# broadinstitute/gatk-bwamem-jni

Hardware: AMD Instinct MI355X
Metric: 150bp reads aligned/sec vs GRCh38-scale reference (1/2/4/8 MI355X) (higher is better)
Workload: dtype u8/int32/int64; 1 GPU; 10000000 x 150bp single-end synthetic reads per GPU vs synthetic GRCh38-scale genome (3100000000 bp, 24 contigs, 5% diverged repeats), full index in HBM; reads_per_gpu=10000000, read_len=150, genome_bp=3100000000, genome=iid, response_bytes=542940344, parallelism=read-sharded x1, no collectives, hip_hw_queues=4, paired_end=False

## Files before the change

gatk-bwamem-jni_amd/csrc/k_seed.hip:

```cpp
#include "dev_common.h"
#include "wave_ops.h"
#include "kernels.h"

DEV uint32_t mask16(int n)
{
    n = n < 0 ? 0 : n > 16 ? 16 : n;
    return (uint32_t)(0x5555555500000000ull >> (n << 1));
}
DEV void cnt_word_m(uint32_t x, uint32_t m, uint32_t& c1, uint32_t& c2, uint32_t& c3)
{
    const uint32_t lo = x & m, hi = (x >> 1) & m;
    c3 += __popc(hi & lo);
    c2 += __popc(hi & ~lo);
    c1 += __popc(~hi & lo);
}
DEV void extend_sm(const DevIndex& ix, uint64_t x0, uint64_t x1, uint64_t size, int c, bool is_back, uint64_t& o0, uint64_t& o1, uint64_t& osz)
{
    const uint64_t xa = is_back ? x0 : x1, xb = is_back ? x1 : x0;
    const uint64_t k = xa - 1, l = xa - 1 + size;
    const uint64_t kk = k - (k >= ix.primary), ll = l - (l >= ix.primary);
    const uint64_t bk = kk >> 6, bl = ll >> 6;
    const uint4* pk = ix.occ + 2 * bk;
    const uint4* pl = ix.occ + 2 * bl;
    const uint4 ck = pk[0], sk = pk[1], cl = pl[0], sl = pl[1];
// ... 291 lines not shown
            i = sx - 1; c = c0;
            if (!walk && (cmask & ~gone & short_mask)) st = S_PRB0;
            else if (lo >= nf) END_SEARCH();
            else { rd = wr = nf - 1; st = S_BWD; }
        }
        if (emit) MEM_PUSH(em0, ems, emi);
        if (ovf) FINISH();
        if (fin) {
            tv.n_intv[r] = ovf ? 0 : mem_n;
            if (ovf) atomicOr(tv.err, ERR_INTV_CAP);
        }
    }
#undef QAT
#undef FINISH
#undef MEM_PUSH
#undef PUSH_IK
#undef END_SEARCH
#undef BEGIN_BWD
    unsigned long long tot = n_ext;
    for (int o = 32; o > 0; o >>= 1) tot += __shfl_down(tot, o);
    if (lane == 0) { count_add(&tv.cnt->n_ext, tot); }
}

__global__ void k_seed_fin(MemOpt opt, TileView tv)
{
    const int r = blockIdx.x * blockDim.x + threadIdx.x;
    if (r >= tv.n_reads) return;
    Intv* a = tv.intv + (size_t)r * tv.intv_cap;
    const int n = tv.n_intv[r];
    for (int i = 1; i < n; ++i) {
        Intv t = a[i];
        int j = i;
        while (j > 0 && a[j - 1].info > t.info) { a[j] = a[j - 1]; --j; }
        a[j] = t;
    }
    int n_seeds = 0, l_rep = 0, b = 0, e = 0;
    int32_t* iso = tv.intv_seed_off + (size_t)r * tv.intv_cap;
    for (int i = 0; i < n; ++i) {
        const Intv p = a[i];
        const int sb = (int)(p.info >> 32), se = (int)(uint32_t)p.info;
        iso[i] = n_seeds;
        {
            int64_t step = p.size > (uint64_t)(int64_t)opt.max_occ ? (int64_t)(p.size / (uint64_t)opt.max_occ) : 1;
            int64_t c = ((int64_t)p.size + step - 1) / step;
            n_seeds += (int)(c < opt.max_occ ? c : opt.max_occ);
        }
        if (p.size <= (uint64_t)(int64_t)opt.max_occ) continue;
        if (sb > e) { l_rep += e - b; b = sb; e = se; }
        else e = e > se ? e : se;
    }
    l_rep += e - b;
    tv.n_seeds[r] = n_seeds;
    tv.l_rep[r] = l_rep;
}

__global__ void __launch_bounds__(1024) k_scan(const int32_t* in, int64_t* out, int n)
{
    __shared__ int64_t wtot[2][16];
    const int t = threadIdx.x, lane = t & 63, wv = t >> 6;
    int64_t carry = 0;
    int ph = 0;
    for (int base = 0; base < n; base += 4096, ph ^= 1) {
        const int i0 = base + t * 4;
        int v0 = 0, v1 = 0, v2 = 0, v3 = 0;
        if (i0 + 3 < n) { const int4 q = *(const int4*)(in + i0); v0 = q.x; v1 = q.y; v2 = q.z; v3 = q.w; }
        else { if (i0 < n) v0 = in[i0]; if (i0 + 1 < n) v1 = in[i0 + 1]; if (i0 + 2 < n) v2 = in[i0 + 2]; }
        const int64_t sum = (int64_t)v0 + v1 + v2 + v3;
        int64_t incl = sum;
        for (int o = 1; o < 64; o <<= 1) { int64_t u = __shfl_up(incl, o); if (lane >= o) incl += u; }
        if (lane == 63) wtot[ph][wv] = incl;
        __syncthreads();
        int64_t pre = carry, tot = 0;
        for (int w = 0; w < 16; ++w) { const int64_t x = wtot[ph][w]; if (w < wv) pre += x; tot += x; }
        int64_t run = pre + incl - sum;
        if (i0 < n) out[i0] = run;
        run += v0; if (i0 + 1 < n) out[i0 + 1] = run;
        run += v1; if (i0 + 2 < n) out[i0 + 2] = run;
        run += v2; if (i0 + 3 < n) out[i0 + 3] = run;
        carry += tot;
    }
    if (t == 0) out[n] = carry;
}

DEV int64_t block_excl_scan_256(int64_t v, int64_t* lds4, int64_t& total)
{
    const int lane = threadIdx.x & 63, wv = threadIdx.x >> 6;
    int64_t incl = v;
    for (int o = 1; o < 64; o <<= 1) { int64_t u = __shfl_up(incl, o); if (lane >= o) incl += u; }
    if (lane == 63) lds4[wv] = incl;
    __syncthreads();
    int64_t pre = 0; total = 0;
    for (int w = 0; w < 4; ++w) { const int64_t x = lds4[w]; if (w < wv) pre += x; total += x; }
    __syncthreads();
    return pre + incl - v;
}
__global__ void __launch_bounds__(256) k_scan_part(const int32_t* in, int n, int64_t* part)
{
    __shared__ int64_t w4[4];
    const int i0 = blockIdx.x * 4096 + threadIdx.x * 16;
    int64_t sum = 0;
    for (int k = 0; k < 16; k += 4) {
        const int i = i0 + k;
        if (i + 3 < n) { const int4 q = *(const int4*)(in + i); sum += (int64_t)q.x + q.y + q.z + q.w; }
        else for (int j = i; j < n && j < i + 4; ++j) sum += in[j];
    }
    int64_t tot;
    (void)block_excl_scan_256(sum, w4, tot);
    if (threadIdx.x == 0) part[blockIdx.x] = tot;
}
__global__ void __launch_bounds__(64) k_scan_top(int64_t* part, int nb, int64_t* total_out)
{
    const int lane = threadIdx.x;
    int64_t carry = 0;
    for (int base = 0; base < nb; base += 64) {
        const int i = base + lane;
        const int64_t v = i < nb ? part[i] : 0;
        int64_t incl = v;
        for (int o = 1; o < 64; o <<= 1) { int64_t u = __shfl_up(incl, o); if (lane >= o) incl += u; }
        if (i < nb) part[i] = carry + incl - v;
        carry += __shfl(incl, 63);
    }
    if (lane == 0) *total_out = carry;
}
template <bool FUSED>
__global__ void __launch_bounds__(256) k_scan_apply(const int32_t* in, int n, const int64_t* part, int64_t* out)
{
    __shared__ int64_t w4[4];
    const int i0 = blockIdx.x * 4096 + threadIdx.x * 16;
    int v[16];
    int64_t sum = 0;
    for (int k = 0; k < 16; ++k) { v[k] = i0 + k < n ? in[i0 + k] : 0; sum += v[k]; }
    int64_t tot, base;
    if (FUSED) {
        int64_t mine = 0, before;
        for (int b = threadIdx.x; b < (int)blockIdx.x; b += 256) mine += part[b];
        (void)block_excl_scan_256(mine, w4, before);
        base = before;
    } else base = part[blockIdx.x];
    int64_t run = base + block_excl_scan_256(sum, w4, tot);
    for (int k = 0; k < 16; ++k) { if (i0 + k < n) out[i0 + k] = run; run += v[k]; }
    if (FUSED && blockIdx.x == gridDim.x - 1 && threadIdx.x == 0) out[n] = base + tot;
}

DEV int order_bin(int n_seeds) { return n_seeds <= 0 ? 31 : __clz(n_seeds); }
__global__ void __launch_bounds__(256) k_order_count(const int32_t* n_seeds, int n, int32_t* bins)
{
    __shared__ int32_t h[32];
    if (threadIdx.x < 32) h[threadIdx.x] = 0;
    __syncthreads();
    const int r = blockIdx.x * blockDim.x + threadIdx.x;
    if (r < n) atomicAdd(&h[order_bin(n_seeds[r])], 1);
    __syncthreads();
    if (threadIdx.x < 32 && h[threadIdx.x]) atomicAdd(&bins[threadIdx.x], h[threadIdx.x]);
}
__global__ void k_order_offsets(int32_t* bins)
{
    if (threadIdx.x == 0 && blockIdx.x == 0) { int acc = 0; for (int b = 0; b < 32; ++b) { bins[32 + b] = acc; acc += bins[b]; } }
}
__global__ void __launch_bounds__(256) k_order_scatter(const int32_t* n_seeds, int n, int32_t* bins, int32_t* order)
{
    __shared__ int32_t h[32], base[32];
    if (threadIdx.x < 32) h[threadIdx.x] = 0;
    __syncthreads();
    const int r = blockIdx.x * blockDim.x + threadIdx.x;
    int b = 0, rank = 0;
    if (r < n) { b = order_bin(n_seeds[r]); rank = atomicAdd(&h[b], 1); }
    __syncthreads();
    if (threadIdx.x < 32) base[threadIdx.x] = h[threadIdx.x] ? atomicAdd(&bins[32 + threadIdx.x], h[threadIdx.x]) : 0;
    __syncthreads();
    if (r < n) order[base[b] + rank] = r;
}
void launch_order(hipStream_t st, const int32_t* n_seeds, int n, int32_t* bins64, int32_t* order)
{
    if (n <= 0) return;
    (void)hipMemsetAsync(bins64, 0, 64 * sizeof(int32_t), st);
    hipLaunchKernelGGL(k_order_count, dim3((n + 255) / 256), dim3(256), 0, st, n_seeds, n, bins64);
    hipLaunchKernelGGL(k_order_offsets, dim3(1), dim3(64), 0, st, bins64);
    hipLaunchKernelGGL(k_order_scatter, dim3((n + 255) / 256), dim3(256), 0, st, n_seeds, n, bins64, order);
}

DEV uint32_t zero_byte_mask(uint32_t w) { return ~(((w & 0x7f7f7f7fu) + 0x7f7f7f7fu) | w | 0x7f7f7f7fu); }
DEV void nul_words(const uint8_t* seq, int64_t n_bytes, int64_t b0, uint32_t m[4])
{
    const uint4 q = *(const uint4*)(seq + b0);
    const uint32_t w[4] = { q.x, q.y, q.z, q.w };
    for (int k = 0; k < 4; ++k) {
        const int64_t left = n_bytes - (b0 + 4 * k);
        uint32_t z = zero_byte_mask(w[k]);
        if (left < 4) z = left <= 0 ? 0u : z & (0xffffffffu >> (8 * (4 - (int)left)));
        m[k] = z;
    }
}
__global__ void __launch_bounds__(256) k_nul_count(const uint8_t* seq, int64_t n_bytes, int32_t* cnt)
{
    __shared__ int64_t w4[4];
    const int64_t b0 = (int64_t)blockIdx.x * 4096 + threadIdx.x * 16;
    uint32_t m[4] = { 0, 0, 0, 0 };
    if (b0 < n_bytes) nul_words(seq, n_bytes, b0, m);
    int64_t tot;
    (void)block_excl_scan_256((int64_t)(__popc(m[0]) + __popc(m[1]) + __popc(m[2]) + __popc(m[3])), w4, tot);
    if (threadIdx.x == 0) cnt[blockIdx.x] = (int32_t)tot;
}
__global__ void __launch_bounds__(256) k_nul_write(const uint8_t* seq, int64_t n_bytes, const int64_t* blk_off, int nb, int64_t* off, int64_t n_reads_max, int64_t* n_found)
{
    __shared__ int64_t w4[4];
    const int64_t b0 = (int64_t)blockIdx.x * 4096 + threadIdx.x * 16;
    uint32_t m[4] = { 0, 0, 0, 0 };
    if (b0 < n_bytes) nul_words(seq, n_bytes, b0, m);
    int64_t tot;
    int64_t k = blk_off[blockIdx.x] + block_excl_scan_256((int64_t)(__popc(m[0]) + __popc(m[1]) + __popc(m[2]) + __popc(m[3])), w4, tot);
    for (int w = 0; w < 4; ++w)
        for (int j = 0; j < 4; ++j)
            if (m[w] >> (8 * j + 7) & 1) { if (k < n_reads_max) off[k + 1] = b0 + 4 * w + j + 1; ++k; }
    if (blockIdx.x == 0 && threadIdx.x == 0) *n_found = blk_off[nb];
}

__global__ void k_sa(DevIndex ix, MemOpt opt, TileView tv, int64_t n_occ)
{
    int64_t g = (int64_t)blockIdx.x * blockDim.x + threadIdx.x;
    uint32_t n_lf = 0, n_sa = 0;
    if (g < n_occ) {
        int lo = 0, hi = tv.n_reads;
        while (hi - lo > 1) { int mid = (lo + hi) >> 1; if (tv.seed_off[mid] <= g) lo = mid; else hi = mid; }
        int r = lo;
        int local = (int)(g - tv.seed_off[r]);
        const int32_t* iso = tv.intv_seed_off + (size_t)r * tv.intv_cap;
        int n = tv.n_intv[r];
        lo = 0; hi = n;
        while (hi - lo > 1) { int mid = (lo + hi) >> 1; if (iso[mid] <= local) lo = mid; else hi = mid; }
        Intv p = tv.intv[(size_t)r * tv.intv_cap + lo];
        int64_t step = p.size > (uint64_t)(int64_t)opt.max_occ ? (int64_t)(p.size / (uint64_t)opt.max_occ) : 1;
        int64_t k = (int64_t)(local - iso[lo]) * step;
        Seed s;
        s.rbeg = (int64_t)sa_lookup(ix, p.x0 + (uint64_t)k, n_lf); ++n_sa;
        s.qbeg = (int32_t)(p.info >> 32);
        s.len = s.score = (int32_t)((uint32_t)p.info - (uint32_t)(p.info >> 32));
        s.next = -1;
        tv.seeds[g] = s;
        tv.seed_rid[g] = bns_intv2rid(ix, s.rbeg, s.rbeg + s.len);
    }
    unsigned long long a = n_lf, b = n_sa;
    for (int o = 32; o > 0; o >>= 1) { a += __shfl_down(a, o); b += __shfl_down(b, o); }
    if ((threadIdx.x & 63) == 0) { count_add(&tv.cnt->n_lf, a); count_add(&tv.cnt->n_sa, b); }
}

__global__ void k_sa_densify(DevIndex ix, const uint64_t* sa_src, uint64_t n_src, int src_intv, uint32_t* lo, uint8_t* hi, int32_t* err)
{
    const uint64_t t = (uint64_t)blockIdx.x * blockDim.x + threadIdx.x;
    if (t >= n_src) return;
    uint64_t k = t * (uint64_t)src_intv, v = sa_src[t];
    lo[k >> ix.sa_shift] = (uint32_t)v; hi[k >> ix.sa_shift] = (uint8_t)(v >> 32);
    if (ix.sa_intv == src_intv) return;
    if (t == 0) v = ix.seq_len;
    const uint64_t smask = (uint64_t)src_intv - 1, dmask = (uint64_t)ix.sa_intv - 1;
    for (uint64_t step = 0; ; ++step) {
        if (step > ix.seq_len) { atomicOr(err, ERR_SCRATCH); return; }
        k = lf_step(ix, k);
        if (!(k & smask)) return;
        --v;
        if (!(k & dmask)) { lo[k >> ix.sa_shift] = (uint32_t)v; hi[k >> ix.sa_shift] = (uint8_t)(v >> 32); }
    }
}

void launch_sa_densify(hipStream_t st, const DevIndex& ix, const uint64_t* sa_src, uint64_t n_src, int src_intv, uint32_t* lo, uint8_t* hi, int32_t* err)
{
    hipLaunchKernelGGL(k_sa_densify, dim3((unsigned)((n_src + 255) / 256)), dim3(256), 0, st, ix, sa_src, n_src, src_intv, lo, hi, err);
}

__global__ void k_build_occ64(const uint32_t* bwt, uint64_t n_blocks, uint4* occ)
{
    uint64_t b = (uint64_t)blockIdx.x * blockDim.x + threadIdx.x;
    if (b >= n_blocks) return;
    const uint32_t* blk = bwt + (b >> 1 << 4);
    const uint64_t* cnt = (const uint64_t*)blk;
    const uint32_t* sym = blk + 8 + ((b & 1) << 2);
    uint32_t c1 = 0, c2 = 0, c3 = 0;
    if (b & 1) for (int i = 0; i < 4; ++i) cnt_word(blk[8 + i], 16, c1, c2, c3);
    const uint64_t C = cnt[1] + c1, G = cnt[2] + c2, T = cnt[3] + c3;
    uint4 c, s;
    c.x = (uint32_t)C; c.y = (uint32_t)G; c.z = (uint32_t)T;
    c.w = (uint32_t)(C >> 32 & 0xff) | (uint32_t)(G >> 32 & 0xff) << 8 | (uint32_t)(T >> 32 & 0xff) << 16;
    s.x = sym[0]; s.y = sym[1]; s.z = sym[2]; s.w = sym[3];
    occ[2 * b] = c; occ[2 * b + 1] = s;
}

void launch_build_occ64(hipStream_t st, const uint32_t* bwt, uint64_t n_blocks, uint4* occ)
{
    hipLaunchKernelGGL(k_build_occ64, dim3((unsigned)((n_blocks + 255) / 256)), dim3(256), 0, st, bwt, n_blocks, occ);
}

__global__ void k_unpack_pac(const uint8_t* pac, int64_t start, int64_t n, uint8_t* dst)
{
    int64_t i = (int64_t)blockIdx.x * blockDim.x + threadIdx.x;
    const int64_t stride = (int64_t)gridDim.x * blockDim.x;
    for (; i < n; i += stride) dst[i] = (uint8_t)pac_base(pac, start + i);
}
void launch_unpack_pac(hipStream_t st, const DevIndex& ix, int64_t start, int64_t n, uint8_t* dst)
{
    if (n <= 0) return;
    int64_t nb = (n + 255) / 256;
    if (nb > 65536) nb = 65536;
    hipLaunchKernelGGL(k_unpack_pac, dim3((unsigned)nb), dim3(256), 0, st, ix.pac, start, n, dst);
}

void launch_encode(hipStream_t st, uint8_t* seq, int64_t n_bytes)
{
    if (n_bytes <= 0) return;
    int64_t nb = (n_bytes + 255) / 256;
    if (nb > 8192) nb = 8192;
    hipLaunchKernelGGL(k_encode, dim3((unsigned)nb), dim3(256), 0, st, seq, n_bytes);
}
void launch_seed(hipStream_t st, const DevIndex& ix, const MemOpt& opt, const TileView& tv)
{
    if (tv.n_reads <= 0) return;
    const int n_cu = ix.n_cu > 0 ? ix.n_cu : 256;
    int K = 16, wpc = 0, refill_min = 4;
    { const char* e = getenv("BWAMEM_HIP_SEED_REFILL"); if (e && atoi(e) > 0) refill_min = atoi(e); }
    { const char* e = getenv("BWAMEM_HIP_SEED_K"); if (e && atoi(e) > 0) K = atoi(e); }
    { const char* e = getenv("BWAMEM_HIP_SEED_WPC"); if (e && atoi(e) > 0) wpc = atoi(e); }
    while (K & (K - 1)) K &= K - 1;
    const size_t qbytes = (size_t)64 * 4 * (((size_t)tv.max_len + 7) / 8);
    const bool ldsq = qbytes <= 24576;
    int narrow = ix.seq_len < (1ull << 35) && tv.max_len < 1023;
    { const char* e = getenv("BWAMEM_HIP_SEED_NARROW"); if (e) narrow = narrow && atoi(e) != 0; }
    const size_t lds = (size_t)(narrow ? 5 * K * 32 : 3 * K * 64) * 4 + (size_t)SEED_EL_CAP * 64 * 4 + (ldsq ? qbytes : 0) + 16;
    if (!wpc) { wpc = (int)((size_t)(160 * 1024) / ((lds + 1023) & ~(size_t)1023)); wpc = wpc < 1 ? 1 : wpc > 16 ? 16 : wpc; }
    const int groups = (tv.n_reads + 63) / 64;
    int grid = groups < n_cu * wpc ? groups : n_cu * wpc;
    if (tv.smem_groups > 0 && grid > tv.smem_groups) grid = tv.smem_groups;
    TileView tvs = tv;
    { const char* e = getenv("BWAMEM_HIP_SEED_PROBE"); if (e && e[0] == '0' && !e[1]) tvs.seed_no_probe = 1; }
    if (ldsq) hipLaunchKernelGGL(k_seed<true>, dim3(grid), dim3(64), lds, st, ix, opt, tvs, K, refill_min, narrow);
    else hipLaunchKernelGGL(k_seed<false>, dim3(grid), dim3(64), lds, st, ix, opt, tvs, K, refill_min, narrow);
    hipLaunchKernelGGL(k_seed_fin, dim3((tv.n_reads + 255) / 256), dim3(256), 0, st, opt, tv);
}
size_t scan_tmp_bytes(int64_t n) { return (size_t)((n + 4095) / 4096 + 2) * 8; }
static int scan_knob(const char* name, int dflt) { const char* e = getenv(name); return e && atoi(e) > 0 ? atoi(e) : dflt; }
void launch_scan(hipStream_t st, const int32_t* in, int64_t* out, int n, int64_t* tmp)
{
    const int single_max = scan_knob("BWAMEM_HIP_SCAN_SINGLE_MAX", 8192), fused_max = scan_knob("BWAMEM_HIP_SCAN_FUSED_MAX", 2048);
    if (n <= single_max || !tmp) { hipLaunchKernelGGL(k_scan, dim3(1), dim3(1024), 0, st, in, out, n); return; }
    const int nb = (n + 4095) / 4096;
    hipLaunchKernelGGL(k_scan_part, dim3(nb), dim3(256), 0, st, in, n, tmp);
    if (nb <= fused_max) { hipLaunchKernelGGL(k_scan_apply<true>, dim3(nb), dim3(256), 0, st, in, n, (const int64_t*)tmp, out); return; }
    hipLaunchKernelGGL(k_scan_top, dim3(1), dim3(64), 0, st, tmp, nb, out + n);
    hipLaunchKernelGGL(k_scan_apply<false>, dim3(nb), dim3(256), 0, st, in, n, (const int64_t*)tmp, out);
}
size_t nul_tmp_bytes(int64_t n_bytes) { const size_t nb = (size_t)((n_bytes + 15) / 4096 + 2); return nb * 4 + 128 + (nb + 1) * 8 + scan_tmp_bytes((int64_t)nb); }
void launch_nul_offsets(hipStream_t st, const uint8_t* seq, int64_t n_bytes, int64_t* off, int64_t n_reads_max, int64_t* n_found, void* tmp)
{
    const int nb = (int)((n_bytes + 4095) / 4096);
    int32_t* cnt = (int32_t*)tmp;
    int64_t* blk_off = (int64_t*)((char*)tmp + (((size_t)(nb + 2) * 4 + 63) & ~(size_t)63));
    int64_t* scan_tmp = blk_off + nb + 1;
    (void)hipMemsetAsync(off, 0, 8, st);
    if (nb <= 0) { (void)hipMemsetAsync(n_found, 0, 8, st); return; }
    hipLaunchKernelGGL(k_nul_count, dim3(nb), dim3(256), 0, st, seq, n_bytes, cnt);
    launch_scan(st, cnt, blk_off, nb, scan_tmp);
    hipLaunchKernelGGL(k_nul_write, dim3(nb), dim3(256), 0, st, seq, n_bytes, (const int64_t*)blk_off, nb, off, n_reads_max, n_found);
}
void launch_sa(hipStream_t st, const DevIndex& ix, const MemOpt& opt, const TileView& tv, int64_t n_occ)
{
    if (n_occ <= 0) return;
    hipLaunchKernelGGL(k_sa, dim3((unsigned)((n_occ + 255) / 256)), dim3(256), 0, st, ix, opt, tv, n_occ);
}
```

gatk-bwamem-jni_amd/csrc/kernels.h:

```cpp
#pragma once
#include <hip/hip_runtime.h>
#include "bwamem_types.h"
#include "bam_encode.h"
#include "bam_sort.h"
#include "bam_dup.h"
#include "fastq_parse.h"

void launch_build_occ64(hipStream_t st, const uint32_t* bwt, uint64_t n_blocks, uint4* occ);
void launch_sa_densify(hipStream_t st, const DevIndex& ix, const uint64_t* sa_src, uint64_t n_src, int src_intv, uint32_t* lo, uint8_t* hi, int32_t* err);
void launch_encode(hipStream_t st, uint8_t* seq, int64_t n_bytes);
void launch_unpack_pac(hipStream_t st, const DevIndex& ix, int64_t start, int64_t n, uint8_t* dst);
void launch_seed(hipStream_t st, const DevIndex& ix, const MemOpt& opt, const TileView& tv);
size_t scan_tmp_bytes(int64_t n);
void launch_scan(hipStream_t st, const int32_t* in, int64_t* out, int n, int64_t* tmp);
void launch_order(hipStream_t st, const int32_t* n_seeds, int n, int32_t* bins64, int32_t* order);
size_t nul_tmp_bytes(int64_t n_bytes);
void launch_nul_offsets(hipStream_t st, const uint8_t* seq, int64_t n_bytes, int64_t* off, int64_t n_reads_max, int64_t* n_found, void* tmp);
void launch_sa(hipStream_t st, const DevIndex& ix, const MemOpt& opt, const TileView& tv, int64_t n_occ);
void launch_chain(hipStream_t st, const DevIndex& ix, const MemOpt& opt, const TileView& tv, Chain* chain_store);
bool rescore_needed(const MemOpt& opt, const TileView& tv);
void launch_rescore(hipStream_t st, const DevIndex& ix, const MemOpt& opt, const TileView& tv, void* jobs, void* results, int32_t* first_num, int32_t* cnt, int cap);
size_t extend_lds_bytes(const MemOpt& opt, int max_len);
void launch_extend(hipStream_t st, const DevIndex& ix, const MemOpt& opt, const TileView& tv);
void launch_post1(hipStream_t st, const DevIndex& ix, const MemOpt& opt, const TileView& tv);
void launch_final_prep(hipStream_t st, const DevIndex& ix, const MemOpt& opt, const TileView& tv);
size_t gcigar_slab_bytes(const MemOpt& opt, int max_len);
int gcigar_slab_grid(const DevIndex& ix, int n_jobs);
void launch_gcigar(hipStream_t st, const DevIndex& ix, const MemOpt& opt, const TileView& tv, int n_jobs, const void* jobs, void* outs, uint32_t* cig_pool, int cig_cap,
                   uint8_t* zpool, unsigned long long zpool_cap, unsigned long long* zpool_cur, uint8_t* slabs, size_t slab_bytes, int* queue);
void launch_final_se(hipStream_t st, const DevIndex& ix, const MemOpt& opt, const TileView& tv, const void* job_out, const uint32_t* job_cig, int cig_cap);
void launch_pack(hipStream_t st, const TileView& tv, uint8_t* dst);
void launch_bam_size(hipStream_t st, const BamTile& t);
void launch_bam_emit(hipStream_t st, const BamTile& t);
void launch_qual_check(hipStream_t st, const uint8_t* raw, const uint8_t* qual, const int64_t* raw_off, int n_reads, int32_t* err);
void launch_mate_names(hipStream_t st, const uint8_t* names, const int64_t* name_off, int n_pairs, int32_t* err);
void launch_fastq_count(hipStream_t st, const uint8_t* text, int64_t n, int32_t* counts);
void launch_fastq_starts(hipStream_t st, const FastqText& t);
void launch_fastq_records(hipStream_t st, const FastqText& t, const FastqOut& o);
void launch_fastq_copy(hipStream_t st, const FastqText& t, const FastqOut& o, int max_len);
int bgzf_grid(int n_cu, int64_t n_blocks);
size_t bgzf_token_bytes(int grid);
void launch_bgzf_deflate(hipStream_t st, const uint8_t* src, int64_t n, int n_blocks, int grid, uint8_t* slots, int32_t* sizes, uint32_t* tokens);
void launch_bgzf_gather(hipStream_t st, const uint8_t* slots, const int32_t* sizes, const int64_t* off, int n_blocks, bool with_eof, uint8_t* out);
void launch_sort_bits(hipStream_t st, const uint64_t* keys, int64_t n, int32_t* bits);
void launch_sort_hist(hipStream_t st, const uint64_t* keys, int64_t n, int byte, int32_t* hist);
void launch_sort_scatter(hipStream_t st, const uint64_t* keys, const uint32_t* idx, int64_t n, int byte, const int64_t* off, uint64_t* keys_out, uint32_t* idx_out);
void launch_bamrec_count(hipStream_t st, const uint8_t* bam, const int64_t* bam_off, int n_reads, int32_t* counts, int32_t* bits, int32_t* err);
void launch_bamrec_keys(hipStream_t st, const uint8_t* bam, const int64_t* bam_off, int n_reads, const int64_t* first, uint64_t* keys, int64_t* src_off, int32_t* sizes);
void launch_bamrec_sizes(hipStream_t st, const uint32_t* idx, const int32_t* sizes, int n, int32_t* out);
void launch_bamrec_gather(hipStream_t st, const uint8_t* src, const int64_t* src_off, const uint32_t* idx, const int64_t* dst_off, int n_rec, int64_t total, uint8_t* dst);
void launch_bai_records(hipStream_t st, const BaiView& v);
void launch_bai_mark(hipStream_t st, const uint64_t* keys, const uint32_t* idx, int n, int32_t* start);
void launch_bai_chunks(hipStream_t st, const uint64_t* keys, const uint32_t* idx, int n, const int32_t* start, const int64_t* cid, const int64_t* rec_off,
                       const int64_t* member_off, int64_t coffset0, BaiChunk* out);
void launch_bai_windows(hipStream_t st, const int32_t* win, int n_win, int n_rec, const int64_t* rec_off, const int64_t* member_off, int64_t coffset0, uint64_t* out);
void launch_dup_entries(hipStream_t st, const DupView& v);
void launch_dup_scores(hipStream_t st, const DupView& v, int max_len);
void launch_dup_score_keys(hipStream_t st, const DupView& v, uint64_t* frag_key, uint64_t* pair_key);
void launch_dup_gather(hipStream_t st, const uint64_t* src, const uint32_t* idx, int n, uint64_t* out);
void launch_dup_decide(hipStream_t st, const uint64_t* keys, const uint32_t* idx, const uint64_t* second, int n, const uint8_t* is_paired, uint8_t* dup);
void launch_dup_flags(hipStream_t st, const DupView& v);

void launch_pestat_cand(hipStream_t st, const DevIndex& ix, const MemOpt& opt, const TileView& tv, int8_t* cand_dir, int64_t* cand_is);
void launch_pe_caps(hipStream_t st, const MemOpt& opt, const TileView& tv, int32_t* caps);
void launch_pe_copy_regs(hipStream_t st, const TileView& tv, const AlnReg* src, const int64_t* src_off, AlnReg* dst, const int64_t* dst_off, const int32_t* n_regs);
void launch_pe_pair(hipStream_t st, const DevIndex& ix, const MemOpt& opt, const TileView& tv, AlnReg* regs, const int64_t* reg_off,
                    int32_t* n_regs, int32_t* ints, void* vpool, void* keys, uint8_t* scratch, int64_t scratch_per_pair, int cap_h, int cap_b, int cap_u, const MemPestat* pes, const PairTab& ptab, void* states,
                    void* rescue_jobs, void* rescue_res, int32_t* rescue_first, int32_t* rescue_num, int32_t* rescue_cnt, int rescue_cap);
size_t pe_rescue_bytes(int what, int cap);
void launch_sw_jobs(hipStream_t st, const DevIndex& ix, const MemOpt& opt, const TileView& tv, const void* jobs, const int32_t* cnt, int cap, void* results, int cap_b, int max_qlen);
void launch_pe_out(hipStream_t st, const DevIndex& ix, const MemOpt& opt, const TileView& tv, AlnReg* regs, const int64_t* reg_off,
                   int32_t* n_regs, int32_t* ints, const MemPestat* pes, const void* states, const void* job_out, const uint32_t* job_cig, int cig_cap);
size_t pe_state_bytes(int n_reads);
```

gatk-bwamem-jni_amd/csrc/pipeline.cpp:

```cpp
#include <hip/hip_runtime.h>
#include <stdio.h>
#include <stdlib.h>
#include <string.h>
#include <math.h>
#include <unistd.h>
#include <fcntl.h>
#include <errno.h>
#include <time.h>
#include <sys/stat.h>
#include <sys/mman.h>
#include <dlfcn.h>
#include <mutex>
#include <condition_variable>
#include <thread>
#include <atomic>
#include <functional>
#include <memory>
#include <string>
#include <vector>
#include <deque>
#include <stdexcept>
#include <algorithm>
#include <cmath>
#include "bwamem_types.h"
// ... 1201 lines not shown
static void pe_candidates(const bwamem_batch_s* b, std::vector<int8_t>& dir, std::vector<int64_t>& is)
{
    dir.clear(); is.clear();
    if (!b->pe) return;
    for (const PeTile& t : b->pe->tiles) { dir.insert(dir.end(), t.cand_dir.begin(), t.cand_dir.end()); is.insert(is.end(), t.cand_is.begin(), t.cand_is.end()); }
}

static bool align_batch_pe(bwaidx_s* ix, const MemOpt& opt, const MemPestat* pes0, bwamem_batch_s* b, int64_t read_id0)
{
    if (!pe_begin(ix, opt, pes0, b, read_id0)) return false;
    if (pes0) return true;
    MemPestat pes[4];
    {
        RoctxRange rr("bwamem_hip:pestat");
        std::vector<int8_t> cand_dir; std::vector<int64_t> cand_is;
        pe_candidates(b, cand_dir, cand_is);
        host_pestat(opt, cand_dir, cand_is, pes);
    }
    return pe_finish(ix, opt, pes, b);
}

static void release_tile_outputs(bwamem_batch_s* b)
{
    for (TileOut& t : b->tiles) { if (t.d && t.owned) (void)hipFree(t.d); if (t.d_off) (void)hipFree(t.d_off); }
    b->tiles.clear(); b->result_bytes = 0; b->aligned = false; b->bam_bytes = 0; b->bgzf.bytes = 0; b->bam_encoded = b->bam_sorted = false;
}


static bool align_batch(bwaidx_s* ix, const MemOpt& opt, const MemPestat* pes, bwamem_batch_s* b, int64_t read_id0, int pe_step = 0)
{
    HIP_OK(hipSetDevice(ix->device));
    Workspace& ws = ix->ws;
    if (!ws.stream) HIP_OK(hipStreamCreate(&ws.stream));
    release_tile_outputs(b);
    b->pe.reset();
    b->sink.begin_call(b->n_reads);
    b->read_id0 = read_id0;
    if (b->n_reads == 0) { b->aligned = pe_step != 1; return true; }
    if (!b->h_payload) {
        HIP_OK(hipMemcpyAsync(b->d_seq.p, b->d_raw.p, b->n_bytes, hipMemcpyDeviceToDevice, ws.stream));
        TIMED(ws, K_ENCODE, launch_encode(ws.stream, b->d_seq.as<uint8_t>(), (int64_t)b->n_bytes));
        HIP_OK(hipStreamSynchronize(ws.stream));
        timed_collect(ws);
        if (!b->sink.to_host && b->sink.last_total && !b->sink.pool.ensure(b->sink.last_total + b->sink.last_total / 16 + 4096)) return false;
    } else b->n_bytes = 0;
    bool ok;
    if (pe_step == 1) ok = pe_begin(ix, opt, nullptr, b, read_id0);
    else if (opt.flag & MEM_F_PE) ok = align_batch_pe(ix, opt, pes, b, read_id0);
    else {
        CallPipe pp;
        pp.on_new_tiles = [&](size_t n) { b->tiles.resize(b->tiles.size() + n); b->sink.add_tiles(n); };
        ok = run_pipeline(ix, opt, b, false, pp, [&](Workspace& w, size_t i, const TileSpec& spec, const SeedStore& store, uint32_t chunk_r0) {
            if (!read_length_ok(ix, spec.L)) return false;
            TileOut* to;
            { std::lock_guard<std::mutex> lk(pp.mu); to = &b->tiles[i]; }
            return run_tile_se(ix, w, opt, b, read_id0, i, spec, *to, store, chunk_r0, w.out_cap_hint);
        });
        if (ok) for (const TileOut& t : b->tiles) b->result_bytes += t.bytes;
    }
    if (ok && pe_step != 1) { b->sink.last_total = b->result_bytes; b->aligned = true; }
    return ok;
}

__attribute__((constructor)) static void hip_runtime_defaults() { setenv("GPU_MAX_HW_QUEUES", "8", 0); }

template <typename R, typename F> static R guarded(const char* what, R fail, F&& f) noexcept
{
    try { return f(); }
    catch (const std::exception& ex) { fprintf(stderr, "[bwamem_hip] %s: %s\n", what, ex.what()); }
    catch (...) { fprintf(stderr, "[bwamem_hip] %s: unknown exception\n", what); }
    return fail;
}

const std::vector<ContigInfo>& bwamem_index_contigs(const bwaidx_t* idx) { return idx->h.contigs; }

extern "C" {

int bwamem_hip_set_device(int device) { g_device = device; g_device_explicit = true; return hipSetDevice(device) == hipSuccess ? 0 : -1; }
int bwamem_hip_device_count(void) { int n = 0; return hipGetDeviceCount(&n) == hipSuccess ? n : 0; }

void bwamem_hip_stats_enable(int on) { g_stats.enabled = on != 0; }
void bwamem_hip_stats_reset(void) { std::lock_guard<std::mutex> lk(g_stats.mu); memset(&g_stats.s, 0, sizeof g_stats.s); }
void bwamem_hip_stats_get(bwamem_stats_t* out) { std::lock_guard<std::mutex> lk(g_stats.mu); *out = g_stats.s; }

void jnibwa_free(void* p) { free(p); }

const char* jnibwa_getVersion(void) { return "bwamem-hip-gfx950 (behavioural target: lh3/bwa cb950614ce7217788780b9a8d445c64cd4d8f62e)"; }

mem_opt_t* jnibwa_createDefaultOptions(void)
{
    MemOpt* o = (MemOpt*)calloc(1, sizeof(MemOpt));
    o->a = 1; o->b = 4; o->o_del = o->o_ins = 6; o->e_del = o->e_ins = 1;
    o->w = 100; o->T = 30; o->zdrop = 100; o->pen_unpaired = 17; o->pen_clip5 = o->pen_clip3 = 5;
    o->max_mem_intv = 20; o->min_seed_len = 19; o->split_width = 10; o->max_occ = 500; o->max_chain_gap = 10000;
    o->max_ins = 10000; o->mask_level = 0.50f; o->drop_ratio = 0.50f; o->XA_drop_ratio = 0.80f; o->split_factor = 1.5f;
    o->chunk_size = 10000000; o->n_threads = 1; o->max_XA_hits = 5; o->max_XA_hits_alt = 200; o->max_matesw = 50;
    o->mask_level_redun = 0.95f; o->min_chain_weight = 0; o->max_chain_extend = 1 << 30;
    o->mapQ_coef_len = 50; o->mapQ_coef_fac = (int)log((double)o->mapQ_coef_len);
    int k = 0;
    for (int i = 0; i < 4; ++i) { for (int j = 0; j < 4; ++j) o->mat[k++] = (int8_t)(i == j ? o->a : -o->b); o->mat[k++] = -1; }
    for (int j = 0; j < 5; ++j) o->mat[k++] = -1;
    return (mem_opt_t*)o;
}

int jnibwa_createReferenceIndex(const char* refFileName, const char* indexPrefix, const char* algoName)
{
    return guarded("jnibwa_createReferenceIndex", 1, [&]() -> int {
        if (algoName && strcmp(algoName, "auto") && strcmp(algoName, "is") && strcmp(algoName, "rb2")) return -1;
        std::string err;
        if (!build_index_files(refFileName, indexPrefix, &err)) { fprintf(stderr, "[bwamem_hip] index build failed: %s\n", err.c_str()); return 1; }
        return 0;
    });
}

int jnibwa_createIndexFile(const char* refName, const char* imgName)
{
    return guarded("jnibwa_createIndexFile", 2, [&]() -> int {
        std::string err;
        std::vector<uint8_t> img = image_from_index_files(refName, &err);
        if (img.empty()) { printf("Failed to load index %s: %s\n", refName, err.c_str()); return 2; }
        int fd = open(imgName, O_WRONLY | O_CREAT | O_TRUNC, 0644);
        if (fd == -1) { printf("Failed to open %s for writing: %s\n", imgName, strerror(errno)); return 2; }
        size_t len = img.size();
        const uint8_t* buf = img.data();
        while (len) {
            size_t to_write = std::min<size_t>(len, (size_t)1 << 30);
            if (write(fd, buf, to_write) != (ssize_t)to_write) { printf("Failed to write %s: %s\n", imgName, strerror(errno)); close(fd); return 2; }
            buf += to_write; len -= to_write;
        }
        if (close(fd) != 0) { printf("Failed to close %s: %s\n", imgName, strerror(errno)); return 2; }
        return 0;
    });
}

static std::vector<int> index_devices()
{
    std::vector<int> v;
    int n = 0;
    if (hipGetDeviceCount(&n) != hipSuccess || n <= 0) n = 0;
    const char* e = getenv("BWAMEM_HIP_DEVICES");
    if (e && *e && strcmp(e, "all")) {
        for (const char* p = e; *p; ) {
            char* end; long d = strtol(p, &end, 10);
            if (end == p) break;
            if (d >= 0 && d < n) v.push_back((int)d);
            p = *end == ',' ? end + 1 : end;
            if (*end && *end != ',') break;
        }
        if (v.empty()) v.push_back(g_device);
        return v;
    }
    if (g_device_explicit && !e) { v.push_back(g_device); return v; }
    for (int d = 0; d < n; ++d) v.push_back(d);
    if (v.empty()) v.push_back(g_device);
    return v;
}

static void destroy_replica(bwaidx_s* ix) { (void)hipSetDevice(ix->device); delete ix; }

bwaidx_t* jnibwa_openIndex(int fd)
{
    return guarded("jnibwa_openIndex", (bwaidx_t*)0, [&]() -> bwaidx_t* {
        struct stat st;
        if (fstat(fd, &st) == -1) { close(fd); return 0; }
        void* mem = mmap(0, (size_t)st.st_size, PROT_READ, MAP_SHARED, fd, 0);
        close(fd);
// ... 991 lines not shown
```

include/bwamem_hip.h:

```cpp
#ifndef BWAMEM_HIP_H_
#define BWAMEM_HIP_H_

#include <stddef.h>
#include <stdint.h>

#ifdef __cplusplus
extern "C" {
#endif

typedef struct bwaidx_s bwaidx_t;
typedef struct mem_opt_s mem_opt_t;
typedef struct mem_pestat_s mem_pestat_t;

int jnibwa_createReferenceIndex(const char* refFileName, const char* indexPrefix, const char* algoName);

int jnibwa_createIndexFile(const char* refName, const char* imgName);

bwaidx_t* jnibwa_openIndex(int fd);

int jnibwa_destroyIndex(bwaidx_t* pIdx);

void* jnibwa_getRefContigNames(bwaidx_t* pIdx, size_t* pBufSize);

void* jnibwa_createAlignments(bwaidx_t* pIdx, mem_opt_t* pOpts, mem_pestat_t* peStats, char* pSeq, size_t* pBufSize);
// ... 5 lines not shown
const char* jnibwa_getVersion(void);


int bwamem_hip_set_device(int device);
int bwamem_hip_device_count(void);
int bwamem_hip_index_replicas(bwaidx_t* idx);

int bwamem_hip_index_contig_lengths(bwaidx_t* idx, int64_t* lens, int cap);
int bwamem_hip_index_unpack_pac(bwaidx_t* idx, int64_t start, int64_t n, void* d_dst);

int bwamem_hip_build_image(const uint8_t* codes, int64_t l_pac, int32_t n_contigs, const char* const* names, const int64_t* lens, const char* img_path);

typedef struct bwamem_batch_s bwamem_batch_t;

bwamem_batch_t* bwamem_hip_batch_upload(bwaidx_t* idx, const char* pSeq, size_t nBytes);
bwamem_batch_t* bwamem_hip_batch_wrap_device(bwaidx_t* idx, const void* d_payload, size_t nBytes, uint32_t nReads, const int64_t* h_offsets);
int bwamem_hip_batch_align(bwaidx_t* idx, const mem_opt_t* opt, const mem_pestat_t* pes, bwamem_batch_t* b, int64_t read_id0);
int bwamem_hip_batch_pe_begin(bwaidx_t* idx, const mem_opt_t* opt, bwamem_batch_t* b, int64_t read_id0);
size_t bwamem_hip_batch_pe_candidates(const bwamem_batch_t* b, int8_t* dir, int64_t* isize);
void bwamem_hip_pestat(const mem_opt_t* opt, const int8_t* dir, const int64_t* isize, size_t n, mem_pestat_t* pes );
int bwamem_hip_batch_pe_finish(bwaidx_t* idx, const mem_opt_t* opt, const mem_pestat_t* pes , bwamem_batch_t* b);
size_t bwamem_hip_batch_result_bytes(const bwamem_batch_t* b);
int bwamem_hip_batch_download(bwamem_batch_t* b, void* dst);
void bwamem_hip_batch_free(bwamem_batch_t* b);

char* bwamem_hip_sam_header(bwaidx_t* idx, size_t* pBytes);
char* bwamem_hip_response_to_sam(bwaidx_t* idx, const char* pSeq, const void* response, size_t responseBytes, const char* const* readNames, int paired, size_t* pBytes);

int    bwamem_hip_batch_keep_offsets(bwamem_batch_t* b, int on);
int    bwamem_hip_batch_encode_bam(bwamem_batch_t* b, int paired, const char* names, const int64_t* name_off);
size_t bwamem_hip_batch_bam_bytes(const bwamem_batch_t* b);
int    bwamem_hip_batch_bam_download(bwamem_batch_t* b, void* dst);
void*  bwamem_hip_bam_header(bwaidx_t* idx, size_t* pBytes);
void*  bwamem_hip_bgzf_compress(const void* src, size_t n, int level, int n_threads, int with_eof, size_t* pBytes);
int    bwamem_hip_align_to_bam(bwaidx_t* idx, const mem_opt_t* opt, const mem_pestat_t* pes, const char* pSeq, size_t nBytes,
                               const char* const* readNames, int level, int fd, int write_header);
int64_t bwamem_hip_bam_record_bytes(const void* rec, size_t n_words, int k, int32_t l_read, int32_t l_name);

int    bwamem_hip_batch_compress_bam(bwamem_batch_t* b, int with_eof);
size_t bwamem_hip_batch_bgzf_bytes(const bwamem_batch_t* b);
int    bwamem_hip_batch_bgzf_download(bwamem_batch_t* b, void* dst);
void*  bwamem_hip_bgzf_compress_device(bwaidx_t* idx, const void* src, size_t n, int with_eof, size_t* pBytes);
int    bwamem_hip_align_to_bam_device(bwaidx_t* idx, const mem_opt_t* opt, const mem_pestat_t* pes, const char* pSeq, size_t nBytes,
                                      const char* const* readNames, int fd, int write_header);

int    bwamem_hip_batch_sort_bam(bwamem_batch_t* b);
void*  bwamem_hip_batch_index_bam(bwamem_batch_t* b, int64_t coffset0, size_t* pBytes);
void*  bwamem_hip_bam_header_sorted(bwaidx_t* idx, size_t* pBytes);
int    bwamem_hip_align_to_sorted_bam(bwaidx_t* idx, const mem_opt_t* opt, const mem_pestat_t* pes, const char* pSeq, size_t nBytes,
                                      const char* const* readNames, int fd, int fd_bai, int write_header);
int    bwamem_hip_sort_pairs_device(bwaidx_t* idx, const uint64_t* keys, size_t n, uint32_t* perm);

int    bwamem_hip_batch_set_qualities(bwamem_batch_t* b, const char* quals, size_t nBytes);
int    bwamem_hip_batch_set_read_group(bwamem_batch_t* b, const char* rg_line);
void*  bwamem_hip_bam_header_rg(bwaidx_t* idx, int sorted, const char* rg_line, size_t* pBytes);
char*  bwamem_hip_sam_header_rg(bwaidx_t* idx, const char* rg_line, size_t* pBytes);
char*  bwamem_hip_response_to_sam_q(bwaidx_t* idx, const char* pSeq, const void* response, size_t responseBytes, const char* const* readNames, int paired,
                                    const char* quals, const char* rgId, size_t* pBytes);
bwamem_batch_t* bwamem_hip_batch_upload_fastq(bwaidx_t* idx, const char* text1, size_t n1, const char* text2, size_t n2, int64_t* bad_record);
int    bwamem_hip_align_fastq_to_bam(bwaidx_t* idx, const mem_opt_t* opt, const mem_pestat_t* pes, const char* text1, size_t n1, const char* text2, size_t n2,
                                     const char* rg_line, int sort, int fd, int fd_bai, int write_header);

typedef struct {
    uint64_t unpaired_reads_examined, read_pairs_examined, secondary_or_supplementary, unmapped_reads, unpaired_read_duplicates, read_pair_duplicates;
} bwamem_dup_counts_t;
int    bwamem_hip_batch_mark_duplicates(bwamem_batch_t* b, int paired, bwamem_dup_counts_t* counts);
int    bwamem_hip_mark_duplicates_device(bwaidx_t* idx, void* records, size_t nBytes, const int64_t* read_off, size_t nReads, int paired,
                                         bwamem_dup_counts_t* counts);
int    bwamem_hip_align_to_marked_bam(bwaidx_t* idx, const mem_opt_t* opt, const mem_pestat_t* pes, const char* pSeq, size_t nBytes,
                                      const char* const* readNames, int sort, int fd, int fd_bai, int write_header, bwamem_dup_counts_t* counts);
int    bwamem_hip_align_fastq_to_marked_bam(bwaidx_t* idx, const mem_opt_t* opt, const mem_pestat_t* pes, const char* text1, size_t n1, const char* text2,
                                            size_t n2, const char* rg_line, int sort, int fd, int fd_bai, int write_header, bwamem_dup_counts_t* counts);

typedef struct {
    uint64_t n_reads, n_ext, n_lf, n_sa, n_dp_cells;
    double ms_encode, ms_seed, ms_sa, ms_chain, ms_extend, ms_post, ms_final, ms_pack, ms_other;
    uint64_t n_launch_seed, n_launch_sa, n_launch_extend;
    uint64_t n_tiles, n_retries;
} bwamem_stats_t;

void bwamem_hip_stats_enable(int on);
void bwamem_hip_stats_reset(void);
void bwamem_hip_stats_get(bwamem_stats_t* out);

#ifdef __cplusplus
}
#endif
#endif
```

Before: 25.27 million reads/s.

## Use single-wave scan/order kernels and granule-aware seed LDS occupancy planning

Rewrites the prefix-scan and read-ordering kernels as single-wavefront blocks that use shuffles and ballots instead of LDS and __syncthreads, with each wave handling 1024 reads. Moves the seed kernel's waves-per-CU calculation into a helper that rounds LDS to a 1280-byte granule and supports an optional reserve, which can allow more waves than the old 1024-byte rounding. The SA kernel launch drops from 256-thread to 64-thread blocks. Also exposes the LDS plan through a new C API function. The ballot loops add serial iterations per distinct bin, and smaller blocks mean more blocks to schedule.

```diff
diff --git a/gatk-bwamem-jni_amd/csrc/k_seed.hip b/gatk-bwamem-jni_amd/csrc/k_seed.hip
--- a/gatk-bwamem-jni_amd/csrc/k_seed.hip
+++ b/gatk-bwamem-jni_amd/csrc/k_seed.hip
@@ -397,6 +397,146 @@
     if (t == 0) out[n] = carry;
 }
 
+DEV int64_t wave_sum64(int64_t v)
+{
+    for (int o = 32; o > 0; o >>= 1) v += __shfl_xor(v, o);
+    return v;
+}
+__global__ void __launch_bounds__(64) k_scan_part(const int32_t* in, int n, int64_t* part)
+{
+    const int lane = threadIdx.x;
+    int64_t sum = 0;
+    for (int k = 0; k < 16; ++k) {
+        const int64_t i = (int64_t)blockIdx.x * 4096 + (k * 64 + lane) * 4;
+        if (i + 3 < n) { const int4 q = *(const int4*)(in + i); sum += (int64_t)q.x + q.y + q.z + q.w; }
+        else for (int64_t j = i; j < n && j < i + 4; ++j) sum += in[j];
+    }
+    sum = wave_sum64(sum);
+    if (lane == 0) part[blockIdx.x] = sum;
+}
+__global__ void __launch_bounds__(64) k_scan_top(int64_t* part, int nb, int64_t* total_out)
+{
+    const int lane = threadIdx.x;
+    int64_t carry = 0;
+    for (int base = 0; base < nb; base += 64) {
+        const int i = base + lane;
+        const int64_t v = i < nb ? part[i] : 0;
+        int64_t incl = v;
+        for (int o = 1; o < 64; o <<= 1) { int64_t u = __shfl_up(incl, o); if (lane >= o) incl += u; }
+        if (i < nb) part[i] = carry + incl - v;
+        carry += __shfl(incl, 63);
+    }
+    if (lane == 0) *total_out = carry;
+}
+template <bool FUSED>
+__global__ void __launch_bounds__(64) k_scan_apply(const int32_t* in, int n, const int64_t* part, int64_t* out)
+{
+    const int lane = threadIdx.x;
+    int64_t run;
+    if (FUSED) {
+        int64_t mine = 0;
+        for (int b = lane; b < (int)blockIdx.x; b += 64) mine += part[b];
+        run = wave_sum64(mine);
+    } else run = part[blockIdx.x];
+    for (int k = 0; k < 16; ++k) {
+        const int64_t i0 = (int64_t)blockIdx.x * 4096 + (k * 64 + lane) * 4;
+        if ((int64_t)blockIdx.x * 4096 + k * 256 >= n) break;
+        int v0 = 0, v1 = 0, v2 = 0, v3 = 0;
+        if (i0 + 3 < n) { const int4 q = *(const int4*)(in + i0); v0 = q.x; v1 = q.y; v2 = q.z; v3 = q.w; }
+        else { if (i0 < n) v0 = in[i0]; if (i0 + 1 < n) v1 = in[i0 + 1]; if (i0 + 2 < n) v2 = in[i0 + 2]; }
+        const int64_t sum = (int64_t)v0 + v1 + v2 + v3;
+        int64_t incl = sum;
+        for (int o = 1; o < 64; o <<= 1) { int64_t u = __shfl_up(incl, o); if (lane >= o) incl += u; }
+        int64_t x = run + incl - sum;
+        if (i0 < n) out[i0] = x;
+        x += v0; if (i0 + 1 < n) out[i0 + 1] = x;
+        x += v1; if (i0 + 2 < n) out[i0 + 2] = x;
+        x += v2; if (i0 + 3 < n) out[i0 + 3] = x;
+        run += __shfl(incl, 63);
+    }
+    if (FUSED && blockIdx.x == gridDim.x - 1 && lane == 0) out[n] = run;
+}
+
+#define ORDER_PER_WAVE 1024
+DEV int order_bin(int n_seeds) { return n_seeds <= 0 ? 31 : __clz(n_seeds); }
+__global__ void __launch_bounds__(64) k_order_count(const int32_t* n_seeds, int n, int32_t* bins)
+{
+    const int lane = threadIdx.x;
+    int cnt = 0;
+    for (int k = 0; k < ORDER_PER_WAVE / 64; ++k) {
+        const int64_t r = (int64_t)blockIdx.x * ORDER_PER_WAVE + k * 64 + lane;
+        const bool valid = r < n;
+        const int b = valid ? order_bin(n_seeds[r]) : -1;
+        unsigned long long todo = wave_ballot(valid);
+        while (todo) {
+            const int bb = __shfl(b, __ffsll((long long)todo) - 1);
+            const unsigned long long m = wave_ballot(b == bb);
+            if (lane == bb) cnt += __popcll(m);
+            todo &= ~m;
+        }
+    }
+    if (lane < 32 && cnt) atomicAdd(&bins[lane], cnt);
+}
+__global__ void k_order_offsets(int32_t* bins)
+{
+    if (threadIdx.x == 0 && blockIdx.x == 0) { int acc = 0; for (int b = 0; b < 32; ++b) { bins[32 + b] = acc; acc += bins[b]; } }
+}
+__global__ void __launch_bounds__(64) k_order_scatter(const int32_t* n_seeds, int n, int32_t* bins, int32_t* order)
+{
+    const int lane = threadIdx.x;
+    const unsigned long long below = (1ull << lane) - 1;
+    int bin[ORDER_PER_WAVE / 64];
+    int cnt = 0;
+#pragma unroll
+    for (int k = 0; k < ORDER_PER_WAVE / 64; ++k) {
+        const int64_t r = (int64_t)blockIdx.x * ORDER_PER_WAVE + k * 64 + lane;
+        const bool valid = r < n;
+        bin[k] = valid ? order_bin(n_seeds[r]) : -1;
+        unsigned long long todo = wave_ballot(valid);
+        while (todo) {
+            const int bb = __shfl(bin[k], __ffsll((long long)todo) - 1);
+            const unsigned long long m = wave_ballot(bin[k] == bb);
+            if (lane == bb) cnt += __popcll(m);
+            todo &= ~m;
+        }
+    }
+    int cur = lane < 32 && cnt ? atomicAdd(&bins[32 + lane], cnt) : 0;
+#pragma unroll
+    for (int k = 0; k < ORDER_PER_WAVE / 64; ++k) {
+        const int64_t r = (int64_t)blockIdx.x * ORDER_PER_WAVE + k * 64 + lane;
+        unsigned long long todo = wave_ballot(bin[k] >= 0);
+        while (todo) {
+            const int bb = __shfl(bin[k], __ffsll((long long)todo) - 1);
+            const unsigned long long m = wave_ballot(bin[k] == bb);
+            const int at = __shfl(cur, bb);
+            if (bin[k] == bb) order[at + __popcll(m & below)] = (int32_t)r;
+            if (lane == bb) cur += __popcll(m);
+            todo &= ~m;
+        }
+    }
+}
+void launch_order(hipStream_t st, const int32_t* n_seeds, int n, int32_t* bins64, int32_t* order)
+{
+    if (n <= 0) return;
+    (void)hipMemsetAsync(bins64, 0, 64 * sizeof(int32_t), st);
+    const int nw = (n + ORDER_PER_WAVE - 1) / ORDER_PER_WAVE;
+    hipLaunchKernelGGL(k_order_count, dim3(nw), dim3(64), 0, st, n_seeds, n, bins64);
+    hipLaunchKernelGGL(k_order_offsets, dim3(1), dim3(64), 0, st, bins64);
+    hipLaunchKernelGGL(k_order_scatter, dim3(nw), dim3(64), 0, st, n_seeds, n, bins64, order);
+}
+
+DEV uint32_t zero_byte_mask(uint32_t w) { return ~(((w & 0x7f7f7f7fu) + 0x7f7f7f7fu) | w | 0x7f7f7f7fu); }
+DEV void nul_words(const uint8_t* seq, int64_t n_bytes, int64_t b0, uint32_t m[4])
+{
+    const uint4 q = *(const uint4*)(seq + b0);
+    const uint32_t w[4] = { q.x, q.y, q.z, q.w };
+    for (int k = 0; k < 4; ++k) {
+        const int64_t left = n_bytes - (b0 + 4 * k);
+        uint32_t z = zero_byte_mask(w[k]);
+        if (left < 4) z = left <= 0 ? 0u : z & (0xffffffffu >> (8 * (4 - (int)left)));
+        m[k] = z;
+    }
+}
 DEV int64_t block_excl_scan_256(int64_t v, int64_t* lds4, int64_t& total)
 {
     const int lane = threadIdx.x & 63, wv = threadIdx.x >> 6;
@@ -408,103 +548,6 @@
     for (int w = 0; w < 4; ++w) { const int64_t x = lds4[w]; if (w < wv) pre += x; total += x; }
     __syncthreads();
     return pre + incl - v;
-}
-__global__ void __launch_bounds__(256) k_scan_part(const int32_t* in, int n, int64_t* part)
-{
-    __shared__ int64_t w4[4];
-    const int i0 = blockIdx.x * 4096 + threadIdx.x * 16;
-    int64_t sum = 0;
-    for (int k = 0; k < 16; k += 4) {
-        const int i = i0 + k;
-        if (i + 3 < n) { const int4 q = *(const int4*)(in + i); sum += (int64_t)q.x + q.y + q.z + q.w; }
-        else for (int j = i; j < n && j < i + 4; ++j) sum += in[j];
-    }
-    int64_t tot;
-    (void)block_excl_scan_256(sum, w4, tot);
-    if (threadIdx.x == 0) part[blockIdx.x] = tot;
-}
-__global__ void __launch_bounds__(64) k_scan_top(int64_t* part, int nb, int64_t* total_out)
-{
-    const int lane = threadIdx.x;
-    int64_t carry = 0;
-    for (int base = 0; base < nb; base += 64) {
-        const int i = base + lane;
-        const int64_t v = i < nb ? part[i] : 0;
-        int64_t incl = v;
-        for (int o = 1; o < 64; o <<= 1) { int64_t u = __shfl_up(incl, o); if (lane >= o) incl += u; }
-        if (i < nb) part[i] = carry + incl - v;
-        carry += __shfl(incl, 63);
-    }
-    if (lane == 0) *total_out = carry;
-}
-template <bool FUSED>
-__global__ void __launch_bounds__(256) k_scan_apply(const int32_t* in, int n, const int64_t* part, int64_t* out)
-{
-    __shared__ int64_t w4[4];
-    const int i0 = blockIdx.x * 4096 + threadIdx.x * 16;
-    int v[16];
-    int64_t sum = 0;
-    for (int k = 0; k < 16; ++k) { v[k] = i0 + k < n ? in[i0 + k] : 0; sum += v[k]; }
-    int64_t tot, base;
-    if (FUSED) {
-        int64_t mine = 0, before;
-        for (int b = threadIdx.x; b < (int)blockIdx.x; b += 256) mine += part[b];
-        (void)block_excl_scan_256(mine, w4, before);
-        base = before;
-    } else base = part[blockIdx.x];
-    int64_t run = base + block_excl_scan_256(sum, w4, tot);
-    for (int k = 0; k < 16; ++k) { if (i0 + k < n) out[i0 + k] = run; run += v[k]; }
-    if (FUSED && blockIdx.x == gridDim.x - 1 && threadIdx.x == 0) out[n] = base + tot;
-}
-
-DEV int order_bin(int n_seeds) { return n_seeds <= 0 ? 31 : __clz(n_seeds); }
-__global__ void __launch_bounds__(256) k_order_count(const int32_t* n_seeds, int n, int32_t* bins)
-{
-    __shared__ int32_t h[32];
-    if (threadIdx.x < 32) h[threadIdx.x] = 0;
-    __syncthreads();
-    const int r = blockIdx.x * blockDim.x + threadIdx.x;
-    if (r < n) atomicAdd(&h[order_bin(n_seeds[r])], 1);
-    __syncthreads();
-    if (threadIdx.x < 32 && h[threadIdx.x]) atomicAdd(&bins[threadIdx.x], h[threadIdx.x]);
-}
-__global__ void k_order_offsets(int32_t* bins)
-{
-    if (threadIdx.x == 0 && blockIdx.x == 0) { int acc = 0; for (int b = 0; b < 32; ++b) { bins[32 + b] = acc; acc += bins[b]; } }
-}
-__global__ void __launch_bounds__(256) k_order_scatter(const int32_t* n_seeds, int n, int32_t* bins, int32_t* order)
-{
-    __shared__ int32_t h[32], base[32];
-    if (threadIdx.x < 32) h[threadIdx.x] = 0;
-    __syncthreads();
-    const int r = blockIdx.x * blockDim.x + threadIdx.x;
-    int b = 0, rank = 0;
-    if (r < n) { b = order_bin(n_seeds[r]); rank = atomicAdd(&h[b], 1); }
-    __syncthreads();
-    if (threadIdx.x < 32) base[threadIdx.x] = h[threadIdx.x] ? atomicAdd(&bins[32 + threadIdx.x], h[threadIdx.x]) : 0;
-    __syncthreads();
-    if (r < n) order[base[b] + rank] = r;
-}
-void launch_order(hipStream_t st, const int32_t* n_seeds, int n, int32_t* bins64, int32_t* order)
-{
-    if (n <= 0) return;
-    (void)hipMemsetAsync(bins64, 0, 64 * sizeof(int32_t), st);
-    hipLaunchKernelGGL(k_order_count, dim3((n + 255) / 256), dim3(256), 0, st, n_seeds, n, bins64);
-    hipLaunchKernelGGL(k_order_offsets, dim3(1), dim3(64), 0, st, bins64);
-    hipLaunchKernelGGL(k_order_scatter, dim3((n + 255) / 256), dim3(256), 0, st, n_seeds, n, bins64, order);
-}
-
-DEV uint32_t zero_byte_mask(uint32_t w) { return ~(((w & 0x7f7f7f7fu) + 0x7f7f7f7fu) | w | 0x7f7f7f7fu); }
-DEV void nul_words(const uint8_t* seq, int64_t n_bytes, int64_t b0, uint32_t m[4])
-{
-    const uint4 q = *(const uint4*)(seq + b0);
-    const uint32_t w[4] = { q.x, q.y, q.z, q.w };
-    for (int k = 0; k < 4; ++k) {
-        const int64_t left = n_bytes - (b0 + 4 * k);
-        uint32_t z = zero_byte_mask(w[k]);
-        if (left < 4) z = left <= 0 ? 0u : z & (0xffffffffu >> (8 * (4 - (int)left)));
-        m[k] = z;
-    }
 }
 __global__ void __launch_bounds__(256) k_nul_count(const uint8_t* seq, int64_t n_bytes, int32_t* cnt)
 {
@@ -625,6 +668,18 @@
     if (nb > 8192) nb = 8192;
     hipLaunchKernelGGL(k_encode, dim3((unsigned)nb), dim3(256), 0, st, seq, n_bytes);
 }
+SeedLdsPlan seed_lds_plan(int max_len, bool narrow, size_t reserve, int K)
+{
+    SeedLdsPlan p;
+    const size_t qbytes = (size_t)64 * 4 * (((size_t)(max_len > 0 ? max_len : 0) + 7) / 8);
+    p.ldsq = qbytes <= 24576;
+    p.bytes = (size_t)(narrow ? 5 * K * 32 : 3 * K * 64) * 4 + (size_t)SEED_EL_CAP * 64 * 4 + (p.ldsq ? qbytes : 0) + 16;
+    p.alloc = (p.bytes + SEED_LDS_GRANULE - 1) / SEED_LDS_GRANULE * SEED_LDS_GRANULE;
+    const size_t room = reserve < SEED_LDS_PER_CU ? SEED_LDS_PER_CU - reserve : 0;
+    const size_t w = room / p.alloc;
+    p.waves = w < 1 ? 1 : w > 16 ? 16 : (int)w;
+    return p;
+}
 void launch_seed(hipStream_t st, const DevIndex& ix, const MemOpt& opt, const TileView& tv)
 {
     if (tv.n_reads <= 0) return;
@@ -634,12 +689,14 @@
     { const char* e = getenv("BWAMEM_HIP_SEED_K"); if (e && atoi(e) > 0) K = atoi(e); }
     { const char* e = getenv("BWAMEM_HIP_SEED_WPC"); if (e && atoi(e) > 0) wpc = atoi(e); }
     while (K & (K - 1)) K &= K - 1;
-    const size_t qbytes = (size_t)64 * 4 * (((size_t)tv.max_len + 7) / 8);
-    const bool ldsq = qbytes <= 24576;
     int narrow = ix.seq_len < (1ull << 35) && tv.max_len < 1023;
     { const char* e = getenv("BWAMEM_HIP_SEED_NARROW"); if (e) narrow = narrow && atoi(e) != 0; }
-    const size_t lds = (size_t)(narrow ? 5 * K * 32 : 3 * K * 64) * 4 + (size_t)SEED_EL_CAP * 64 * 4 + (ldsq ? qbytes : 0) + 16;
-    if (!wpc) { wpc = (int)((size_t)(160 * 1024) / ((lds + 1023) & ~(size_t)1023)); wpc = wpc < 1 ? 1 : wpc > 16 ? 16 : wpc; }
+    size_t reserve = 0;
+    { const char* e = getenv("BWAMEM_HIP_SEED_RESERVE"); if (e && atoi(e) > 0) reserve = (size_t)atoi(e); }
+    const SeedLdsPlan plan = seed_lds_plan(tv.max_len, narrow != 0, reserve, K);
+    const size_t lds = plan.bytes;
+    const bool ldsq = plan.ldsq;
+    if (!wpc) wpc = plan.waves;
     const int groups = (tv.n_reads + 63) / 64;
     int grid = groups < n_cu * wpc ? groups : n_cu * wpc;
     if (tv.smem_groups > 0 && grid > tv.smem_groups) grid = tv.smem_groups;
@@ -656,10 +713,10 @@
     const int single_max = scan_knob("BWAMEM_HIP_SCAN_SINGLE_MAX", 8192), fused_max = scan_knob("BWAMEM_HIP_SCAN_FUSED_MAX", 2048);
     if (n <= single_max || !tmp) { hipLaunchKernelGGL(k_scan, dim3(1), dim3(1024), 0, st, in, out, n); return; }
     const int nb = (n + 4095) / 4096;
-    hipLaunchKernelGGL(k_scan_part, dim3(nb), dim3(256), 0, st, in, n, tmp);
-    if (nb <= fused_max) { hipLaunchKernelGGL(k_scan_apply<true>, dim3(nb), dim3(256), 0, st, in, n, (const int64_t*)tmp, out); return; }
+    hipLaunchKernelGGL(k_scan_part, dim3(nb), dim3(64), 0, st, in, n, tmp);
+    if (nb <= fused_max) { hipLaunchKernelGGL(k_scan_apply<true>, dim3(nb), dim3(64), 0, st, in, n, (const int64_t*)tmp, out); return; }
     hipLaunchKernelGGL(k_scan_top, dim3(1), dim3(64), 0, st, tmp, nb, out + n);
-    hipLaunchKernelGGL(k_scan_apply<false>, dim3(nb), dim3(256), 0, st, in, n, (const int64_t*)tmp, out);
+    hipLaunchKernelGGL(k_scan_apply<false>, dim3(nb), dim3(64), 0, st, in, n, (const int64_t*)tmp, out);
 }
 size_t nul_tmp_bytes(int64_t n_bytes) { const size_t nb = (size_t)((n_bytes + 15) / 4096 + 2); return nb * 4 + 128 + (nb + 1) * 8 + scan_tmp_bytes((int64_t)nb); }
 void launch_nul_offsets(hipStream_t st, const uint8_t* seq, int64_t n_bytes, int64_t* off, int64_t n_reads_max, int64_t* n_found, void* tmp)
@@ -677,5 +734,5 @@
 void launch_sa(hipStream_t st, const DevIndex& ix, const MemOpt& opt, const TileView& tv, int64_t n_occ)
 {
     if (n_occ <= 0) return;
-    hipLaunchKernelGGL(k_sa, dim3((unsigned)((n_occ + 255) / 256)), dim3(256), 0, st, ix, opt, tv, n_occ);
-}
+    hipLaunchKernelGGL(k_sa, dim3((unsigned)((n_occ + 63) / 64)), dim3(64), 0, st, ix, opt, tv, n_occ);
+}
diff --git a/gatk-bwamem-jni_amd/csrc/kernels.h b/gatk-bwamem-jni_amd/csrc/kernels.h
--- a/gatk-bwamem-jni_amd/csrc/kernels.h
+++ b/gatk-bwamem-jni_amd/csrc/kernels.h
@@ -11,6 +11,10 @@
 void launch_encode(hipStream_t st, uint8_t* seq, int64_t n_bytes);
 void launch_unpack_pac(hipStream_t st, const DevIndex& ix, int64_t start, int64_t n, uint8_t* dst);
 void launch_seed(hipStream_t st, const DevIndex& ix, const MemOpt& opt, const TileView& tv);
+#define SEED_LDS_PER_CU ((size_t)160 * 1024)
+#define SEED_LDS_GRANULE ((size_t)1280)
+struct SeedLdsPlan { size_t bytes, alloc; int waves; bool ldsq; };
+SeedLdsPlan seed_lds_plan(int max_len, bool narrow, size_t reserve, int K = 16);
 size_t scan_tmp_bytes(int64_t n);
 void launch_scan(hipStream_t st, const int32_t* in, int64_t* out, int n, int64_t* tmp);
 void launch_order(hipStream_t st, const int32_t* n_seeds, int n, int32_t* bins64, int32_t* order);
diff --git a/gatk-bwamem-jni_amd/csrc/pipeline.cpp b/gatk-bwamem-jni_amd/csrc/pipeline.cpp
--- a/gatk-bwamem-jni_amd/csrc/pipeline.cpp
+++ b/gatk-bwamem-jni_amd/csrc/pipeline.cpp
@@ -1307,6 +1307,13 @@
 void bwamem_hip_stats_enable(int on) { g_stats.enabled = on != 0; }
 void bwamem_hip_stats_reset(void) { std::lock_guard<std::mutex> lk(g_stats.mu); memset(&g_stats.s, 0, sizeof g_stats.s); }
 void bwamem_hip_stats_get(bwamem_stats_t* out) { std::lock_guard<std::mutex> lk(g_stats.mu); *out = g_stats.s; }
+int bwamem_hip_seed_lds_plan(int max_len, int narrow, int reserve_bytes, int* bytes, int* alloc_bytes)
+{
+    const SeedLdsPlan p = seed_lds_plan(max_len, narrow != 0, reserve_bytes > 0 ? (size_t)reserve_bytes : 0);
+    if (bytes) *bytes = (int)p.bytes;
+    if (alloc_bytes) *alloc_bytes = (int)p.alloc;
+    return p.waves;
+}
 
 void jnibwa_free(void* p) { free(p); }
 
diff --git a/include/bwamem_hip.h b/include/bwamem_hip.h
--- a/include/bwamem_hip.h
+++ b/include/bwamem_hip.h
@@ -111,6 +111,7 @@
 void bwamem_hip_stats_enable(int on);
 void bwamem_hip_stats_reset(void);
 void bwamem_hip_stats_get(bwamem_stats_t* out);
+int bwamem_hip_seed_lds_plan(int max_len, int narrow, int reserve_bytes, int* bytes, int* alloc_bytes);
 
 #ifdef __cplusplus
 }
```

Result: no change. 25.26 million reads/s (median of 2 runs) (-0.0%).
